# dominikh/jello

Hardware: AMD Instinct MI355X
Metric: Mpixels/sec fine-raster + paths/sec, 100k-path 4096^2 scene (higher is better)
Workload: dtype f32

## Files before the change

jello_amd/csrc/kernels_flatten.hip:

```cpp
#include <hip/hip_runtime.h>
__shared__ double fl_atan_tab[9];
#define JD_ATAN_TAB_LDS fl_atan_tab
#include "kcommon.h"
#define FF_INLINE __device__ __forceinline__
#include "flatten_fast.h"

using namespace jk;
using namespace jd;

namespace {

struct CubicParams { float th0, th1, chord_len, err; };
struct EulerParams { float th0, th1, k0, k1, ch; };
struct CubicPoints { V2 p0, p1, p2, p3; };
struct PointDeriv { V2 point, deriv; };
struct PathTagData { uint32_t tag_byte; MonoidK<5> monoid; };

#define DERIV_THRESH 1e-6f
#define DERIV_THRESH_SQUARED (DERIV_THRESH * DERIV_THRESH)
#define DERIV_EPS 1e-6f
#define SUBDIV_LIMIT (1.0f / 65536.0f)
#define K1_THRESH 1e-3f
#define DIST_THRESH 1e-3f
#define TANGENT_THRESH 1e-6f
// ... 684 lines not shown
            if (tag_monoids.ok(word_ix)) {
                store_tm(&tag_monoids.p[word_ix], pm);
            } else {
#pragma unroll
                for (int i = 0; i < 5; i++) pm.v[i] = 0u;
            }
            __syncthreads();
        } else {
            pm = load_tm(tag_monoids, word_ix);
        }
        const uint32_t ix0 = word_ix * 4u;
        for (uint32_t q = 0u; q < 12u; q++) {
            const uint32_t sl = ix0 * 3u + q;
            if (sl < cap) counts[sl] = 0u;
        }
        uint32_t th = 0u, tl = 0u;
#pragma unroll
        for (uint32_t k = 0; k < 4u; k++) {
            const uint32_t ix = ix0 + k;
            if (ix >= n_tags) continue;
            const MonoidK<5> tm = monoid_add(pm, reduce_tag(tag_word & ((1u << (k * 8u)) - 1u)));
            const uint32_t tag_byte = (tag_word >> (k * 8u)) & 0xffu;
            const uint32_t style_flags = scene.rd(cfg->layout.style_base + tm.v[3] - 2u);
            const bool is_stroke = (style_flags & JL_STYLE_FLAGS_STYLE) != 0u;
            const uint32_t path_ix = tm.v[4];
            if ((tag_byte & JL_PATH_TAG_PATH) != 0u && path_bboxes.ok(path_ix)) {
                path_bboxes.p[path_ix].draw_flags = ((style_flags & JL_STYLE_FLAGS_FILL) == 0u) ? 0u : 1u;
                path_bboxes.p[path_ix].trans_ix = tm.v[0] - 1u;
            }
            const uint32_t seg_type = tag_byte & JL_PATH_TAG_SEG_TYPE;
            const bool curved = seg_type != JL_PATH_TAG_LINETO;
            if (seg_type != 0u) {
                if (!is_stroke) {
                    if (curved) nh[blk][k] = 1u; else nl[blk][k] = 1u;
                } else if ((tag_byte & JL_PATH_TAG_SUBPATH_END) != 0u) {
                    if (curved) nl[blk][k] = 1u;
                } else {
                    if (curved) { nh[blk][k] = 2u; nl[blk][k] = 1u; } else { nl[blk][k] = 3u; }
                }
            }
            th += nh[blk][k];
            tl += nl[blk][k];
        }
        MonoidK<2> m, tot;
        m.v[0] = th; m.v[1] = tl;
        const MonoidK<2> e2 = block_excl_scan_monoid<2>(m, sh, &tot);
        eh[blk] = wg_h + e2.v[0];
        el[blk] = wg_l + e2.v[1];
        wg_h += tot.v[0];
        wg_l += tot.v[1];
        __syncthreads();
    }
    if (threadIdx.x == 0) {
        sh_base[0] = wg_h ? atomicAdd(&counters[0], wg_h) : 0u;
        sh_base[1] = wg_l ? atomicAdd(&counters[FL_CTR_LIGHT], wg_l) : 0u;
    }
    __syncthreads();
#pragma unroll
    for (uint32_t blk = 0; blk < PSC_BLOCKS; blk++) {
        const uint32_t ix0 = ((blockIdx.x * PSC_BLOCKS + blk) * JL_WG + threadIdx.x) * 4u;
        uint32_t ph = sh_base[0] + eh[blk], pl = sh_base[1] + el[blk];
#pragma unroll
        for (uint32_t k = 0; k < 4u; k++) {
            const uint32_t ix = ix0 + k;
            uint32_t sub = 0u;
            for (uint32_t q = 0; q < nh[blk][k]; q++, sub++, ph++)
                if (ph < cap) list[ph] = ix * 3u + sub;
            for (uint32_t q = 0; q < nl[blk][k]; q++, sub++, pl++)
                if (pl < cap) list[cap - 1u - pl] = ix * 3u + sub;
        }
    }
}

template <bool EMIT>
JD void run_item(const JlConfig* cfg, const Scene& s, Out<EMIT>& o, uint32_t slot, EulerJob& job, uint32_t& path_ix_out) {
    uint32_t ix = slot / 3u, sub = slot - ix * 3u;
    Seg g = load_seg(s, ix);
    uint32_t path_ix = g.tag.monoid.v[4];
    path_ix_out = path_ix;
    uint32_t style_ix = g.tag.monoid.v[3];
    uint32_t trans_ix = g.tag.monoid.v[0];
    uint32_t style_flags = g.style_flags;
    job.path_ix = path_ix; job.trans_ix = trans_ix;
    Xf transform;
    {
        uint32_t base = cfg->layout.transform_base + trans_ix * 6u;
        transform.m0 = u2f(s.scene.rd(base)); transform.m1 = u2f(s.scene.rd(base + 1u)); transform.m2 = u2f(s.scene.rd(base + 2u));
        transform.m3 = u2f(s.scene.rd(base + 3u)); transform.t0 = u2f(s.scene.rd(base + 4u)); transform.t1 = u2f(s.scene.rd(base + 5u));
    }
    CubicPoints pts = read_path_segment(s, g.tag, g.is_stroke);
    if (g.is_stroke) {
        float linewidth = u2f(s.scene.rd(cfg->layout.style_base + style_ix + 1u));
        float offset = 0.5f * linewidth;
        bool is_stroke_cap_marker = (g.tag.tag_byte & JL_PATH_TAG_SUBPATH_END) != 0u;
        if (is_stroke_cap_marker) {
            V2 tangent = cubic_start_tangent(pts.p0, pts.p1, pts.p2, pts.p3);
            V2 offset_tangent = offset * normalize(tangent);
            V2 n = v2(offset_tangent.y * -1.0f, offset_tangent.x * 1.0f);
            draw_cap<EMIT>(o, path_ix, (style_flags & JL_STYLE_FLAGS_START_CAP_MASK) >> 2, pts.p0, pts.p0 - n, pts.p0 + n, -offset_tangent,
                           transform);
        } else {
            const float TT = TANGENT_THRESH * TANGENT_THRESH;
            V2 tan_prev = cubic_end_tangent(pts.p0, pts.p1, pts.p2, pts.p3);
            if (dot(tan_prev, tan_prev) < TT) tan_prev = v2(TANGENT_THRESH, 0.0f);
            V2 offset_tangent = offset * normalize(tan_prev);
            V2 n_prev = v2(offset_tangent.y * -1.0f, offset_tangent.x * 1.0f);
            if (sub < 2u) {
                V2 tan_start = cubic_start_tangent(pts.p0, pts.p1, pts.p2, pts.p3);
                if (dot(tan_start, tan_start) < TT) tan_start = v2(TANGENT_THRESH, 0.0f);
                V2 n_start = offset * normalize(v2(-tan_start.y, tan_start.x));
                job.valid = true; job.cubic = pts; job.local_to_device = transform;
                if (sub == 0u) { job.offset = offset; job.start_p = pts.p0 + n_start; job.end_p = pts.p3 + n_prev; }
                else { job.offset = -offset; job.start_p = pts.p0 - n_start; job.end_p = pts.p3 - n_prev; }
            } else {
                PathTagData ntag = compute_tag_monoid(s, ix + 1u);
                CubicPoints npts = read_path_segment(s, ntag, true);
                bool n_is_closed = (ntag.tag_byte & JL_PATH_TAG_SEG_TYPE) == JL_PATH_TAG_LINETO;
                bool n_is_marker = (ntag.tag_byte & JL_PATH_TAG_SUBPATH_END) != 0u;
                bool do_join = !n_is_marker || n_is_closed;
                if (do_join) {
                    V2 tan_next = cubic_start_tangent(npts.p0, npts.p1, npts.p2, npts.p3);
                    if (dot(tan_next, tan_next) < TT) tan_next = v2(TANGENT_THRESH, 0.0f);
                    V2 tnn = normalize(tan_next);
                    V2 n_next = v2((offset * tnn.y) * -1.0f, (offset * tnn.x) * 1.0f);
                    draw_join<EMIT>(o, path_ix, style_flags, pts.p3, tan_prev, tan_next, n_prev, n_next, transform);
                } else {
                    draw_cap<EMIT>(o, path_ix, (style_flags & JL_STYLE_FLAGS_END_CAP_MASK), pts.p3, pts.p3 + n_prev, pts.p3 - n_prev, offset_tangent,
                                   transform);
                }
            }
        }
    } else {
        job.valid = true; job.cubic = pts; job.local_to_device = transform;
        job.offset = 0.0f; job.start_p = pts.p0; job.end_p = pts.p3;
    }
}

#ifndef FLQ_STACK
#define FLQ_STACK 448u
#endif
#ifndef FLQ_LEAVES
#define FLQ_LEAVES 640u
#endif
#ifndef FLQ_MAX_LEVEL
#define FLQ_MAX_LEVEL 9u
#endif
struct FlBatch {
    uint32_t jhead[64];
    uint32_t stack[FLQ_STACK];
    uint32_t l_tpos[FLQ_LEAVES];
    uint16_t l_key[FLQ_LEAVES];
    uint16_t l_link[FLQ_LEAVES];
    uint32_t unsure[128];
    uint32_t n_stack, n_leaves, bail, n_unsure;
};
JD float lanef(float v, uint32_t src) { return u2f((uint32_t)__builtin_amdgcn_ds_bpermute((int)(src << 2), (int)f2u(v))); }
JD uint32_t laneu(uint32_t v, uint32_t src) { return (uint32_t)__builtin_amdgcn_ds_bpermute((int)(src << 2), (int)v); }

struct NodeResult {
    bool accept;
    CubicParams cp;
    V2 es_p0, es_p1;
    bool ends_at_one;
};
struct NodeEnds {
    V2 last_p, last_q;
    float last_t;
    V2 point, deriv;
    float t1;
};
JD NodeEnds node_ends(V2 p0, V2 p1, V2 p2, V2 p3, uint32_t level, uint32_t t0_u) {
    const float dt = u2f((127u - level) << 23);
    const float t0 = (float)t0_u * dt;
    NodeEnds r;
    if (t0_u == 0u) {
        r.last_p = p0;
        r.last_q = p1 - p0;
        if (dot(r.last_q, r.last_q) < DERIV_THRESH_SQUARED) r.last_q = eval_cubic_and_deriv(p0, p1, p2, p3, DERIV_EPS).deriv;
        r.last_t = 0.0f;
    } else {
        PointDeriv pq0 = eval_cubic_and_deriv(p0, p1, p2, p3, t0);
        r.last_t = t0;
        if (dot(pq0.deriv, pq0.deriv) < DERIV_THRESH_SQUARED) {
            PointDeriv n0 = eval_cubic_and_deriv(p0, p1, p2, p3, t0 - DERIV_EPS);
            pq0.deriv = n0.deriv;
            pq0.point = n0.point;
            r.last_t = t0 - DERIV_EPS;
        }
        r.last_p = pq0.point;
        r.last_q = pq0.deriv;
    }
    float t1 = t0 + dt;
    PointDeriv this_pq1 = eval_cubic_and_deriv(p0, p1, p2, p3, t1);
    if (dot(this_pq1.deriv, this_pq1.deriv) < DERIV_THRESH_SQUARED) {
        PointDeriv new_pq1 = eval_cubic_and_deriv(p0, p1, p2, p3, t1 - DERIV_EPS);
        this_pq1.deriv = new_pq1.deriv;
        if (t1 < 1.0f) {
            this_pq1.point = new_pq1.point;
            t1 = t1 - DERIV_EPS;
        }
    }
    r.point = this_pq1.point;
    r.deriv = this_pq1.deriv;
    r.t1 = t1;
    return r;
}
JD NodeResult node_test(V2 p0, V2 p1, V2 p2, V2 p3, float scale, uint32_t level, uint32_t t0_u) {
    const float tol = 0.25f;
    const float dt = u2f((127u - level) << 23);
    const NodeEnds ne = node_ends(p0, p1, p2, p3, level, t0_u);
    const float actual_dt = ne.t1 - ne.last_t;
    NodeResult r;
    r.cp = cubic_from_points_derivs(ne.last_p, ne.point, ne.last_q, ne.deriv, actual_dt);
    r.accept = r.cp.err * scale <= tol || dt <= SUBDIV_LIMIT;
    r.es_p0 = ne.last_p;
    r.es_p1 = ne.point;
    r.ends_at_one = ne.t1 == 1.0f;
    return r;
}
JD int node_test_fast(V2 p0, V2 p1, V2 p2, V2 p3, float scale, uint32_t level, uint32_t t0_u, float* v_est, float* delta) {
    const float tol = 0.25f;
    const NodeEnds ne = node_ends(p0, p1, p2, p3, level, t0_u);
    const float actual_dt = ne.t1 - ne.last_t;
    const V2 chord = ne.point - ne.last_p;
    const float chord_squared = dot(chord, chord);
    const V2 q0 = ne.last_q, q1 = ne.deriv;
    *v_est = 0.0f; *delta = 0.0f;
    if (chord_squared < DERIV_THRESH_SQUARED) {
        const float chord_err = sqrt_((float)(9.0 / 32.0) * (dot(q0, q0) + dot(q1, q1))) * actual_dt;
        return (chord_err * scale <= tol) ? ffast::FF_ACCEPT : ffast::FF_REJECT;
    }
    const float chord_len = FF_SQRT(chord_squared);
    const float sc = actual_dt * FF_RCP(chord_squared);
    const V2 h0 = v2(q0.x * chord.x + q0.y * chord.y, q0.y * chord.x - q0.x * chord.y);
    const V2 h1 = v2(q1.x * chord.x + q1.y * chord.y, q1.x * chord.y - q1.y * chord.x);
    const float len0 = FF_SQRT(h0.x * h0.x + h0.y * h0.y), len1 = FF_SQRT(h1.x * h1.x + h1.y * h1.y);
    return ffast::ff_decide(h0.x, h0.y, len0, h1.x, h1.y, len1, len0 * sc, len1 * sc, chord_len, scale, tol, v_est, delta);
}
JD CubicParams piece_angles(const NodeEnds& ne) {
    const V2 chord = ne.point - ne.last_p;
    const float chord_squared = dot(chord, chord);
    CubicParams r;
    r.err = 0.0f;
    if (chord_squared < DERIV_THRESH_SQUARED) {
        r.th0 = 0.0f; r.th1 = 0.0f; r.chord_len = DERIV_THRESH;
        return r;
    }
    const V2 q0 = ne.last_q, q1 = ne.deriv;
    const V2 h0 = v2(q0.x * chord.x + q0.y * chord.y, q0.y * chord.x - q0.x * chord.y);
    const V2 h1 = v2(q1.x * chord.x + q1.y * chord.y, q1.x * chord.y - q1.y * chord.x);
    r.th0 = atan2_(h0.y, h0.x);
    r.th1 = atan2_(h1.y, h1.x);
    r.chord_len = sqrt_(chord_squared);
    return r;
}

struct PieceParams {
    EulerParams ep;
    float n, noff, int0, integral;
    uint32_t n_u, robust;
};
JD PieceParams piece_params(const CubicParams& cp, float scale, float offset) {
    const float tol = 0.25f;
    PieceParams r;
    r.ep = es_params_from_angles(cp.th0, cp.th1);
    const EulerParams& ep = r.ep;
    float k0 = ep.k0 - 0.5f * ep.k1;
    float k1 = ep.k1;
    float normalized_offset = offset / cp.chord_len;
    float dist_scaled = normalized_offset * ep.ch;
    float scale_multiplier = sqrt_(0.125f * scale * cp.chord_len / (ep.ch * tol));
    float a = 0.0f, b = 0.0f, integral = 0.0f, int0 = 0.0f, n_frac;
    uint32_t robust = 0u;
    if (abs_(k1) < K1_THRESH) {
        float k = ep.k0;
        n_frac = sqrt_(abs_(k * (k * dist_scaled + 1.0f)));
        robust = 1u;
    } else if (abs_(dist_scaled) < DIST_THRESH) {
        a = k1;
        b = k0;
        int0 = pow_1_5_signed(b);
        float int1 = pow_1_5_signed(a + b);
        integral = int1 - int0;
        n_frac = (float)(2.0 / 3.0) * integral / a;
        robust = 2u;
    } else {
        a = -2.0f * dist_scaled * k1;
        b = -1.0f - 2.0f * dist_scaled * k0;
        int0 = espc_int_approx(b);
        float int1 = espc_int_approx(a + b);
        integral = int1 - int0;
        float k_peak = k0 - k1 * b / a;
        float integrand_peak = sqrt_(abs_(k_peak * (k_peak * dist_scaled + 1.0f)));
        n_frac = integral * integrand_peak / a;
    }
    r.n = clamp_(ceil_(n_frac * scale_multiplier), 1.0f, 100.0f);
    r.n_u = to_u32(r.n);
    r.noff = normalized_offset;
    r.int0 = int0;
    r.integral = integral;
    r.robust = robust;
    return r;
}

#ifdef FL_FAST_CHECK
__device__ uint32_t g_ff_stats[8];
#endif
#ifndef FL_WAVES_PER_EU
#define FL_WAVES_PER_EU 4
#endif
#ifndef FL_BLOCKS_PER_CU
#define FL_BLOCKS_PER_CU 4
#endif
#ifdef FL_TIMING
#define FL_TL_WAVES 8192u
#define FL_TL_BATCHES 15u
#define FL_TL_WORDS (2u + 3u * FL_TL_BATCHES)
__device__ unsigned long long g_fl_timeline[FL_TL_WAVES * FL_TL_WORDS];
#endif
__global__ __launch_bounds__(JL_WG) __attribute__((amdgpu_waves_per_eu(FL_WAVES_PER_EU, FL_WAVES_PER_EU))) void k_flatten_items(const JlConfig* __restrict__ cfg, Buf<uint32_t> scene, Buf<JlTagMonoid> tag_monoids,
                                                         Buf<JlPathBbox> path_bboxes, const uint32_t* __restrict__ list,
                                                         uint32_t* __restrict__ counters, uint32_t cap, uint32_t* __restrict__ counts,
                                                         FlTemp T, uint32_t debug) {
    __shared__ FlBatch sh_batch[JL_WG / 64];
    Scene s;
    s.cfg = cfg; s.scene = scene; s.tag_monoids = tag_monoids;
    uint32_t n_heavy = umin_(counters[0], cap), n_light = umin_(counters[FL_CTR_LIGHT], cap - n_heavy);
    uint32_t n = n_heavy + n_light;
    const uint32_t units_h = n_heavy / 64u + (n_heavy % 64u != 0u ? 1u : 0u);
    const uint32_t units = units_h + n_light / 64u + (n_light % 64u != 0u ? 1u : 0u);
    const uint32_t n_groups = umin_(umax_(gridDim.x / FL_BLOCKS_PER_CU, 1u), FL_DEAL_GROUPS), group = blockIdx.x % n_groups;
    if (group >= units) return;
#ifdef FL_TIMING
    const unsigned long long tl_entry = wall_clock64();
    const uint32_t tl_wave = blockIdx.x * (JL_WG / 64u) + (threadIdx.x >> 6);
    uint32_t tl_n = 0u;
#endif
    atan_tab_fill();
    __syncthreads();
    const uint32_t lane = lane_id();
    FlBatch& B = sh_batch[threadIdx.x >> 6];
    Out<true> o;
    o.cfg = cfg; o.T = T; o.home_s = o.home_r = blockIdx.x % T.K; o.failed_s = o.failed_r = false; o.slot = 0u;
    if ((debug & 1u) != 0u) o.home_s = o.home_r = 0u;
#ifdef FL_SOAK_HOME0
    o.home_s = o.home_r = 0u;
#endif
    o.cursor = 0u; o.a_first = 0u; o.a_spos = 0u; o.a_rpos = 0u;
    for (;;) {
        uint32_t k = 0u;
        if (lane == 0u) k = atomicAdd(&counters[FL_CTR_DEAL + FL_DEAL_STRIDE * group], 1u);
        k = (uint32_t)__builtin_amdgcn_readfirstlane((int)k);
        const uint32_t u = k * n_groups + group;
        if (u >= units) break;
        const bool heavy = u < units_h;
        const uint32_t t_first = heavy ? u * 64u : n_heavy + (u - units_h) * 64u;
        const uint32_t t_end = umin_(t_first + 64u, heavy ? n_heavy : n);
        const uint32_t t = t_first + lane;
#ifdef FL_TIMING
        const unsigned long long tl_start = wall_clock64() | (heavy ? 1ull << 63 : 0ull);
        uint32_t tl_info = 0u;
#define FL_TL_END()                                                                                      \
    do {                                                                                                 \
        if (lane == 0u && tl_wave < FL_TL_WAVES && tl_n < FL_TL_BATCHES) {                               \
            g_fl_timeline[tl_wave * FL_TL_WORDS + 2u + 3u * tl_n] = tl_start;                            \
            g_fl_timeline[tl_wave * FL_TL_WORDS + 3u + 3u * tl_n] = wall_clock64();                      \
            g_fl_timeline[tl_wave * FL_TL_WORDS + 4u + 3u * tl_n] = tl_info;                             \
        }                                                                                                \
        tl_n++;                                                                                          \
    } while (0)
#else
#define FL_TL_END() do {} while (0)
#endif
        if (__builtin_amdgcn_ballot_w64(o.failed_s) != 0ull) { o.home_s = fl_next_home(T, o.home_s, 0); o.failed_s = false; }
        if (__builtin_amdgcn_ballot_w64(o.failed_r) != 0ull) { o.home_r = fl_next_home(T, o.home_r, 1); o.failed_r = false; }
        EulerJob job;
        job.valid = false; job.path_ix = 0u; job.trans_ix = 0u; job.offset = 0.0f;
        job.start_p = v2(0, 0); job.end_p = v2(0, 0);
        job.cubic.p0 = job.cubic.p1 = job.cubic.p2 = job.cubic.p3 = v2(0, 0);
        job.local_to_device = xf_identity();
        uint32_t slot = FL_INVALID;
        if (t < t_end) {
            slot = heavy ? list[t] : list[cap - 1u - (t - n_heavy)];
            o.slot = slot; o.cursor = 0u; o.a_first = 0u; o.a_spos = 0u; o.a_rpos = 0u;
            uint32_t path_ix;
            run_item<true>(cfg, s, o, slot, job, path_ix);
            if (!job.valid) counts[slot] = o.cursor;
        }
        EulerLane e;
        euler_begin(e, job);
        const bool active = job.valid && !e.done;
        if (__builtin_amdgcn_ballot_w64(active) == 0ull) {
            FL_TL_END();
            continue;
        }
        B.jhead[lane] = 0u;
        {
            const uint64_t am = __builtin_amdgcn_ballot_w64(active);
            if (active) B.stack[(uint32_t)__builtin_popcountll(am & ((1ull << lane) - 1ull))] = lane;
            if (lane == 0u) { B.n_stack = (uint32_t)__builtin_popcountll(am); B.n_leaves = 0u; B.bail = 0u; B.n_unsure = 0u; }
        }
        wave_fence();
#ifdef FL_SPLIT_NO_A
        if (lane == 0u) B.n_stack = 0u;
        wave_fence();
#endif
        for (;;) {
#ifdef FL_TIMING
            tl_info += 1u << 16;
#endif
            const uint32_t ns = (uint32_t)__builtin_amdgcn_readfirstlane((int)B.n_stack);
            const uint32_t nu = (uint32_t)__builtin_amdgcn_readfirstlane((int)B.n_unsure);
            if (ns == 0u && nu == 0u) break;
            const bool exact_round = ns == 0u || nu >= 64u;
            const uint32_t take = umin_(exact_round ? nu : ns, 64u);
            const bool has = lane < take;
            const uint32_t node = has ? (exact_round ? B.unsure[nu - 1u - lane] : B.stack[ns - 1u - lane]) : 0u;
            wave_fence();
            const uint32_t j = node & 63u, level = (node >> 6) & 31u, t0_u = node >> 11;
            const V2 jp0 = v2(lanef(e.p0.x, j), lanef(e.p0.y, j)), jp1 = v2(lanef(e.p1.x, j), lanef(e.p1.y, j));
            const V2 jp2 = v2(lanef(e.p2.x, j), lanef(e.p2.y, j)), jp3 = v2(lanef(e.p3.x, j), lanef(e.p3.y, j));
            const float scale = lanef(e.scale, j);
            int kind = ffast::FF_UNSURE;
            if (exact_round) {
                if (has) kind = node_test(jp0, jp1, jp2, jp3, scale, level, t0_u).accept ? ffast::FF_ACCEPT : ffast::FF_REJECT;
            } else if (has) {
                float v_est, delta;
                kind = node_test_fast(jp0, jp1, jp2, jp3, scale, level, t0_u, &v_est, &delta);
#ifdef FL_FAST_CHECK
            }
            if (!exact_round) {
                bool c_unsure = false, c_contra = false, c_viol = false;
                if (has) {
                    float v2_, d2_;
                    const int k2 = node_test_fast(jp0, jp1, jp2, jp3, scale, level, t0_u, &v2_, &d2_);
                    const NodeResult rx = node_test(jp0, jp1, jp2, jp3, scale, level, t0_u);
                    const float vx = rx.cp.err * scale;
                    c_unsure = k2 == ffast::FF_UNSURE;
                    c_contra = (k2 == ffast::FF_ACCEPT && !rx.accept) || (k2 == ffast::FF_REJECT && rx.accept);
                    c_viol = (d2_ > 0.0f && !(abs_(v2_ - vx) <= d2_)) || (d2_ == 0.0f && k2 != ffast::FF_UNSURE && v2_ != 0.0f);
                }
                const uint32_t n0 = (uint32_t)__builtin_popcountll(__builtin_amdgcn_ballot_w64(has));
                const uint32_t n1 = (uint32_t)__builtin_popcountll(__builtin_amdgcn_ballot_w64(c_unsure));
                const uint32_t n2 = (uint32_t)__builtin_popcountll(__builtin_amdgcn_ballot_w64(c_contra));
                const uint32_t n3 = (uint32_t)__builtin_popcountll(__builtin_amdgcn_ballot_w64(c_viol));
                if (lane == 0u) {
                    atomicAdd(&g_ff_stats[0], n0);
                    if (n1) atomicAdd(&g_ff_stats[1], n1);
                    if (n2) atomicAdd(&g_ff_stats[2], n2);
                    if (n3) atomicAdd(&g_ff_stats[3], n3);
                }
#endif
            }
            const bool acc = has && kind == ffast::FF_ACCEPT, rej = has && kind == ffast::FF_REJECT, uns = has && kind == ffast::FF_UNSURE;
            const uint64_t accm = __builtin_amdgcn_ballot_w64(acc), rejm = __builtin_amdgcn_ballot_w64(rej), unsm = __builtin_amdgcn_ballot_w64(uns);
            const uint32_t n_acc = (uint32_t)__builtin_popcountll(accm), n_rej = (uint32_t)__builtin_popcountll(rejm);
            const uint32_t n_uns = (uint32_t)__builtin_popcountll(unsm);
            const uint32_t nl = (uint32_t)__builtin_amdgcn_readfirstlane((int)B.n_leaves);
            const uint32_t ns_left = exact_round ? ns : ns - take, nu_left = exact_round ? nu - take : nu;
            const bool too_deep = __builtin_amdgcn_ballot_w64(rej && level + 1u > FLQ_MAX_LEVEL) != 0ull;
            if (too_deep || ns_left + 2u * n_rej > FLQ_STACK || nl + n_acc > FLQ_LEAVES) {
                if (lane == 0u) B.bail = 1u;
                wave_fence();
                break;
            }
            const uint64_t below = (1ull << lane) - 1ull;
            if (rej) {
                const uint32_t pos = ns_left + 2u * (uint32_t)__builtin_popcountll(rejm & below);
                B.stack[pos] = j | ((level + 1u) << 6) | ((2u * t0_u + 1u) << 11);
                B.stack[pos + 1u] = j | ((level + 1u) << 6) | ((2u * t0_u) << 11);
            }
            if (acc) {
                const uint32_t li = nl + (uint32_t)__builtin_popcountll(accm & below);
                B.l_tpos[li] = node;
                B.l_key[li] = (uint16_t)((t0_u << (FLQ_MAX_LEVEL - level)) << 7);
                const uint32_t prev = atomicExch(&B.jhead[j], li + 1u);
                B.l_link[li] = (uint16_t)((j << 10) | prev);
            }
            if (uns) B.unsure[nu_left + (uint32_t)__builtin_popcountll(unsm & below)] = node;
            if (lane == 0u) { B.n_stack = ns_left + 2u * n_rej; B.n_leaves = nl + n_acc; B.n_unsure = nu_left + n_uns; }
            wave_fence();
        }
        const bool bail = (uint32_t)__builtin_amdgcn_readfirstlane((int)B.bail) != 0u;
        const uint32_t nl = bail ? 0u : (uint32_t)__builtin_amdgcn_readfirstlane((int)B.n_leaves);
#ifdef FL_TIMING
        tl_info = (tl_info & 0x7fff0000u) | (nl & 0xffffu) | (bail ? 1u << 31 : 0u);
#endif
        uint32_t rec_base = 0u;
        if (nl != 0u && lane == 0u) rec_base = fl_grab<1>(T, o.home_r, nl, o.failed_r);
        rec_base = (uint32_t)__builtin_amdgcn_readlane((int)rec_base, 0);
#ifdef FL_SPLIT_NO_B
        for (uint32_t lbase = nl; lbase < nl; lbase += 64u) {
#else
        for (uint32_t lbase = 0u; lbase < nl; lbase += 64u) {
#endif
            const uint32_t li = lbase + lane;
            const bool has = li < nl;
            const uint32_t node = has ? B.l_tpos[li] : 0u;
            const uint32_t j = node & 63u, level = (node >> 6) & 31u, t0_u = node >> 11;
            const V2 jp0 = v2(lanef(e.p0.x, j), lanef(e.p0.y, j)), jp1 = v2(lanef(e.p1.x, j), lanef(e.p1.y, j));
            const V2 jp2 = v2(lanef(e.p2.x, j), lanef(e.p2.y, j)), jp3 = v2(lanef(e.p3.x, j), lanef(e.p3.y, j));
            const float scale = lanef(e.scale, j), offset = lanef(e.offset, j);
            const uint32_t j_slot = laneu(slot, j), j_path = laneu(e.path_ix, j), j_trans = laneu(e.trans_ix, j);
            const float j_tsx = lanef(e.t_start.x, j), j_tsy = lanef(e.t_start.y, j), j_tex = lanef(e.t_end.x, j), j_tey = lanef(e.t_end.y, j);
            if (has) {
                const NodeEnds ne = node_ends(jp0, jp1, jp2, jp3, level, t0_u);
                const CubicParams cp = piece_angles(ne);
                const PieceParams pp = piece_params(cp, scale, offset);
                const uint32_t fl = pp.robust | ((ne.t1 == 1.0f) ? 4u : 0u) | ((offset >= 0.0f) ? 8u : 0u) | ((offset == 0.0f) ? 16u : 0u) |
                                    ((t0_u == 0u) ? 32u : 0u);
                const uint32_t r = rec_base + li;
                if (rec_base != FL_INVALID)
                    piece_record_write(T.recs + (size_t)r * 4u, ne.last_p, ne.point, pp.ep.th0, pp.ep.th1, pp.int0, pp.integral, pp.noff, j_slot, j_path,
                                       j_trans, fl, 0u, v2(j_tsx, j_tsy), v2(j_tex, j_tey));
                B.l_key[li] = (uint16_t)(B.l_key[li] | pp.n_u);
            }
        }
        wave_fence();
        if (nl != 0u) {
            uint32_t total = 0u;
            if (active)
                for (uint32_t q = B.jhead[lane]; q != 0u; q = B.l_link[q - 1u] & 1023u) total += B.l_key[q - 1u] & 127u;
            if (active) counts[slot] = total;
            const uint32_t incl = wave_incl_scan_u32(total);
            const uint32_t batch_total = (uint32_t)__builtin_amdgcn_readlane((int)incl, 63);
            const bool together = batch_total <= ((debug & 4u) != 0u ? 48u : FL_MAX_GRAB);
            uint32_t grab = 0u;
            if (together) {
                if (lane == 0u) grab = fl_grab<0>(T, o.home_s, batch_total, o.failed_s);
            } else if (active && total != 0u) {
                grab = fl_grab<0>(T, o.home_s, total, o.failed_s);
            }
            for (uint32_t li = lane; li < nl; li += 64u) {
                const uint32_t j = B.l_link[li] >> 10, key = B.l_key[li];
                uint32_t first = 0u;
                for (uint32_t q = B.jhead[j]; q != 0u; q = B.l_link[q - 1u] & 1023u) {
                    const uint32_t k2 = B.l_key[q - 1u];
                    if ((k2 >> 7) < (key >> 7)) first += k2 & 127u;
                }
                B.l_tpos[li] = first;
            }
            {
                const uint32_t base0 = (uint32_t)__builtin_amdgcn_readlane((int)grab, 0);
                B.unsure[lane] = together ? (base0 == FL_INVALID ? FL_INVALID : base0 + (incl - total)) : grab;
            }
            wave_fence();
            for (uint32_t li = lane; li < nl; li += 64u) {
                const uint32_t j = B.l_link[li] >> 10, key = B.l_key[li], first = B.l_tpos[li];
                const uint32_t r = rec_base + li, jb = B.unsure[j];
                if (rec_base != FL_INVALID && (key >> 7) != 0u) ((uint32_t*)T.recs)[(size_t)r * 16u + 12u] = first;
                if (jb == FL_INVALID) continue;
                if (rec_base != FL_INVALID) piece_slots_write(T.sinfo, jb + first, key & 127u, r);
                else for (uint32_t i = 0u; i < (key & 127u); i++) T.sinfo[jb + first + i] = make_uint2(0u, 0u);
            }
            wave_fence();
        }
        if (__builtin_expect(bail, 0)) {
            o.slot = slot; o.cursor = 0u; o.a_first = 0u; o.a_spos = 0u; o.a_rpos = 0u;
            bool have = active;
            auto finish = [&]() -> bool {
                if (e.done && have) {
                    counts[o.slot] = o.cursor;
                    have = false;
                }
                return __builtin_amdgcn_ballot_w64(!e.done) != 0ull;
            };
            flatten_euler_wave(o, e, finish);
        }
        FL_TL_END();
    }
#ifdef FL_TIMING
    if (lane == 0u && tl_wave < FL_TL_WAVES) {
        g_fl_timeline[tl_wave * FL_TL_WORDS] = tl_entry;
        g_fl_timeline[tl_wave * FL_TL_WORDS + 1u] = tl_n;
    }
#endif
#undef FL_TL_END
}

#ifndef FL_LINES_WAVES_PER_EU
#define FL_LINES_WAVES_PER_EU 4
#endif
__global__ __launch_bounds__(JL_WG) __attribute__((amdgpu_waves_per_eu(FL_LINES_WAVES_PER_EU, FL_LINES_WAVES_PER_EU))) void k_flatten_lines(const JlConfig* __restrict__ cfg, Buf<uint32_t> scene, const uint32_t* __restrict__ counters,
                                                         FlTemp T, const uint32_t* __restrict__ bases, uint32_t n_slots, Buf<JlLineSoup> lines) {
    atan_tab_fill();
    const uint32_t lines_lim = umin_(cfg->lines_size, lines.n);
    const uint2* __restrict__ sinfo = T.sinfo;
    const uint4* __restrict__ recs = T.recs;
    const uint32_t n_r = T.K * T.R;
    uint32_t ru[FL_MAX_REGIONS], used[FL_MAX_REGIONS];
    uint32_t units = 0u;
#pragma unroll
    for (uint32_t c = 0u; c < FL_MAX_REGIONS; c++) {
        ru[c] = units;
        used[c] = c < T.K ? umin_(counters[FL_CTR_CURSOR + FL_CUR_STRIDE * c], T.R) : 0u;
        units += (used[c] + JL_WG - 1u) / JL_WG;
    }
    auto fetch_info = [&](uint32_t u) -> uint2 {
        if (u >= units) return make_uint2(0u, 0u);
        uint32_t c = 0u, first_unit = 0u, in_use = used[0];
#pragma unroll
        for (uint32_t q = 1u; q < FL_MAX_REGIONS; q++)
            if (u >= ru[q] && used[q] != 0u) { c = q; first_unit = ru[q]; in_use = used[q]; }
        const uint32_t in_region = (u - first_unit) * JL_WG + threadIdx.x;
        return in_region < in_use ? sinfo[(size_t)c * T.R + in_region] : make_uint2(0u, 0u);
    };
    auto state_of = [&](uint2 si) -> uint32_t {
        if (si.x >= n_r) return 0u;
        return (si.y & FL_INFO_PIECE) != 0u ? 2u : ((si.y & FL_INFO_DIRECT) != 0u ? 1u : 0u);
    };
    auto fetch_rec = [&](uint32_t state, uint32_t r, uint4& r0, uint4& r1, uint4& r2, uint4& r3) {
        r0 = r1 = r2 = r3 = make_uint4(0u, 0u, 0u, 0u);
        const uint4* rec = recs + (size_t)r * 4u;
        if (state != 0u) { r0 = rec[0]; r1 = rec[1]; }
        if (state == 2u) { r2 = rec[2]; r3 = rec[3]; }
    };
    const uint32_t G = gridDim.x;
    uint2 si_a = fetch_info(blockIdx.x), si_b = fetch_info(blockIdx.x + G);
    uint32_t st_a = state_of(si_a);
    uint4 a0, a1, a2, a3;
    fetch_rec(st_a, si_a.x, a0, a1, a2, a3);
    for (uint32_t u = blockIdx.x; u < units; u += G) {
        const uint32_t st = st_a;
        const uint2 si = si_a;
        const uint4 r0 = a0, r1 = a1, r2 = a2, r3 = a3;
        si_a = si_b;
        st_a = state_of(si_a);
        fetch_rec(st_a, si_a.x, a0, a1, a2, a3);
        si_b = fetch_info(u + 2u * G);
        uint32_t widx[3] = {0xffffffffu, 0xffffffffu, 0xffffffffu};
        uint2 wdat[3] = {make_uint2(0u, 0u), make_uint2(0u, 0u), make_uint2(0u, 0u)};
        if (st == 1u) {
            const uint32_t item = r0.x, k = r0.y;
            if (item < n_slots) {
                const uint32_t dst = bases[item] + k;
                if (dst < lines_lim) {
                    widx[0] = dst * 3u; wdat[0] = make_uint2(r0.z, 0u);
                    widx[1] = dst * 3u + 1u; wdat[1] = make_uint2(r1.x, r1.y);
                    widx[2] = dst * 3u + 2u; wdat[2] = make_uint2(r1.z, r1.w);
                }
            }
        } else if (st == 2u) {
            const uint32_t n_u = (si.y >> 8) & 127u, i = si.y & 127u;
            const uint32_t flags = r2.w & 63u;
            const bool last_of_item = i + 1u == n_u && (flags & 4u) != 0u;
            const uint32_t slot = r2.y, k = ((flags & 32u) != 0u ? 0u : r3.x) + i;
            Xf tr;
            if ((flags & 16u) != 0u) {
                tr = xf_identity();
            } else {
                uint32_t tb = cfg->layout.transform_base + (r2.w >> 6) * 6u;
                tr.m0 = u2f(scene.rd(tb)); tr.m1 = u2f(scene.rd(tb + 1u)); tr.m2 = u2f(scene.rd(tb + 2u));
                tr.m3 = u2f(scene.rd(tb + 3u)); tr.t0 = u2f(scene.rd(tb + 4u)); tr.t1 = u2f(scene.rd(tb + 5u));
            }
            const uint32_t slot_base = slot < n_slots ? bases[slot] : 0u;
            V2 lp1;
            if (last_of_item) {
                lp1 = v2(u2f(r3.z), u2f(r3.w));
#if defined(FL_LSPLIT) && FL_LSPLIT == 1
            } else if (true) {
                lp1 = v2(u2f(r0.x) + (float)i, u2f(r0.w) + u2f(r1.x) + u2f(r1.y) + u2f(r1.z) + u2f(r1.w) + u2f(r2.x));
#endif
            } else {
                const EulerParams ep = es_params_from_angles(u2f(r1.x), u2f(r1.y));
                const float noff = u2f(r2.x), n = (float)n_u;
                const float tt = (float)(i + 1u) / n;
                float sarg = tt;
                const uint32_t robust = flags & 3u;
                if (robust != 1u) {
                    const float k0 = ep.k0 - 0.5f * ep.k1, k1 = ep.k1;
                    const float dist_scaled = noff * ep.ch;
                    const float int0 = u2f(r1.z), integral = u2f(r1.w);
                    float a, b;
                    if (robust == 2u) {
                        a = k1;
                        b = k0;
                    } else {
                        a = -2.0f * dist_scaled * k1;
                        b = -1.0f - 2.0f * dist_scaled * k0;
                    }
                    float uu = integral * tt + int0;
                    float inv;
                    if (robust == 2u) inv = pow23_abs_(uu) * sign_(uu); else inv = espc_int_inv_approx(uu);
                    sarg = (inv - b) / a;
                }
                lp1 = es_seg_eval_with_offset(v2(u2f(r0.x), u2f(r0.y)), v2(u2f(r0.z), u2f(r0.w)), ep, sarg, noff);
            }
            const V2 q = xf_apply(tr, lp1);
            if (slot < n_slots) {
                const uint32_t dst = slot_base + k;
                const bool fwd = (flags & 8u) != 0u;
                const bool has_next = !last_of_item && dst + 1u < lines_lim;
                const uint2 hdr = make_uint2(r2.z, 0u), pt = make_uint2(f2u(q.x), f2u(q.y));
                if (dst < lines_lim) {
                    if (k == 0u) {
                        uint2* w = (uint2*)lines.p;
                        const V2 qs = xf_apply(tr, v2(u2f(r3.x), u2f(r3.y)));
                        w[(size_t)dst * 3u] = hdr;
                        w[(size_t)dst * 3u + (fwd ? 1u : 2u)] = make_uint2(f2u(qs.x), f2u(qs.y));
                    }
                    widx[0] = dst * 3u + (fwd ? 2u : 1u); wdat[0] = pt;
                    if (has_next) {
// ... 263 lines not shown
```

Before: 20930.

## Share subdivision tree between paired stroke sides in batched flatten

Detects adjacent lanes whose slots form a stroke pair (same cubic with opposite offsets) and lets only the first lane drive the adaptive subdivision tree, tagging its nodes with a pair bit. Accepted leaves of paired trees are emitted twice into a split leaf array (pairs from the front, singles from the back), and the per-leaf endpoint/angle/Euler parameters are computed once and reused for both offsets. This removes duplicated subdivision and curve-fitting work for stroke sides, at the cost of more complex leaf indexing, an extra inner loop over sides, and an assumption that paired sides always subdivide identically.

```diff
diff --git a/jello_amd/csrc/kernels_flatten.hip b/jello_amd/csrc/kernels_flatten.hip
--- a/jello_amd/csrc/kernels_flatten.hip
+++ b/jello_amd/csrc/kernels_flatten.hip
@@ -860,7 +860,7 @@
     uint16_t l_key[FLQ_LEAVES];
     uint16_t l_link[FLQ_LEAVES];
     uint32_t unsure[128];
-    uint32_t n_stack, n_leaves, bail, n_unsure;
+    uint32_t n_stack, n_pairs, n_single, bail, n_unsure;
 };
 JD float lanef(float v, uint32_t src) { return u2f((uint32_t)__builtin_amdgcn_ds_bpermute((int)(src << 2), (int)f2u(v))); }
 JD uint32_t laneu(uint32_t v, uint32_t src) { return (uint32_t)__builtin_amdgcn_ds_bpermute((int)(src << 2), (int)v); }
@@ -968,16 +968,27 @@
     float n, noff, int0, integral;
     uint32_t n_u, robust;
 };
-JD PieceParams piece_params(const CubicParams& cp, float scale, float offset) {
+struct PieceShared {
+    EulerParams ep;
+    float chord_len, scale_multiplier;
+};
+JD PieceShared piece_shared(const CubicParams& cp, float scale) {
     const float tol = 0.25f;
+    PieceShared r;
+    r.ep = es_params_from_angles(cp.th0, cp.th1);
+    r.chord_len = cp.chord_len;
+    r.scale_multiplier = sqrt_(0.125f * scale * cp.chord_len / (r.ep.ch * tol));
+    return r;
+}
+JD PieceParams piece_params(const PieceShared& ps, float offset) {
     PieceParams r;
-    r.ep = es_params_from_angles(cp.th0, cp.th1);
+    r.ep = ps.ep;
     const EulerParams& ep = r.ep;
     float k0 = ep.k0 - 0.5f * ep.k1;
     float k1 = ep.k1;
-    float normalized_offset = offset / cp.chord_len;
+    float normalized_offset = offset / ps.chord_len;
     float dist_scaled = normalized_offset * ep.ch;
-    float scale_multiplier = sqrt_(0.125f * scale * cp.chord_len / (ep.ch * tol));
+    float scale_multiplier = ps.scale_multiplier;
     float a = 0.0f, b = 0.0f, integral = 0.0f, int0 = 0.0f, n_frac;
     uint32_t robust = 0u;
     if (abs_(k1) < K1_THRESH) {
@@ -1067,7 +1078,7 @@
         const uint32_t t = t_first + lane;
 #ifdef FL_TIMING
         const unsigned long long tl_start = wall_clock64() | (heavy ? 1ull << 63 : 0ull);
-        uint32_t tl_info = 0u;
+        unsigned long long tl_info = 0u;
 #define FL_TL_END()                                                                                      \
     do {                                                                                                 \
         if (lane == 0u && tl_wave < FL_TL_WAVES && tl_n < FL_TL_BATCHES) {                               \
@@ -1105,8 +1116,13 @@
         B.jhead[lane] = 0u;
         {
             const uint64_t am = __builtin_amdgcn_ballot_w64(active);
-            if (active) B.stack[(uint32_t)__builtin_popcountll(am & ((1ull << lane) - 1ull))] = lane;
-            if (lane == 0u) { B.n_stack = (uint32_t)__builtin_popcountll(am); B.n_leaves = 0u; B.bail = 0u; B.n_unsure = 0u; }
+            const uint32_t slot_before = laneu(slot, (lane + 63u) & 63u);
+            const bool second = active && lane != 0u && slot - (slot / 3u) * 3u == 1u && slot_before + 1u == slot && ((am >> (lane - 1u)) & 1ull) != 0ull;
+            const uint64_t secm = __builtin_amdgcn_ballot_w64(second), rootm = am & ~secm;
+            const bool two = (((secm >> 1) >> lane) & 1ull) != 0ull;
+            if (active && !second)
+                B.stack[(uint32_t)__builtin_popcountll(rootm & ((1ull << lane) - 1ull))] = lane | (two ? 0x80000000u : 0u);
+            if (lane == 0u) { B.n_stack = (uint32_t)__builtin_popcountll(rootm); B.n_pairs = 0u; B.n_single = 0u; B.bail = 0u; B.n_unsure = 0u; }
         }
         wave_fence();
 #ifdef FL_SPLIT_NO_A
@@ -1123,9 +1139,12 @@
             const bool exact_round = ns == 0u || nu >= 64u;
             const uint32_t take = umin_(exact_round ? nu : ns, 64u);
             const bool has = lane < take;
+#ifdef FL_TIMING
+            if (!exact_round) tl_info += (unsigned long long)take << 32;
+#endif
             const uint32_t node = has ? (exact_round ? B.unsure[nu - 1u - lane] : B.stack[ns - 1u - lane]) : 0u;
             wave_fence();
-            const uint32_t j = node & 63u, level = (node >> 6) & 31u, t0_u = node >> 11;
+            const uint32_t j = node & 63u, level = (node >> 6) & 31u, t0_u = (node >> 11) & 0xfffffu;
             const V2 jp0 = v2(lanef(e.p0.x, j), lanef(e.p0.y, j)), jp1 = v2(lanef(e.p1.x, j), lanef(e.p1.y, j));
             const V2 jp2 = v2(lanef(e.p2.x, j), lanef(e.p2.y, j)), jp3 = v2(lanef(e.p3.x, j), lanef(e.p3.y, j));
             const float scale = lanef(e.scale, j);
@@ -1164,10 +1183,13 @@
             const uint64_t accm = __builtin_amdgcn_ballot_w64(acc), rejm = __builtin_amdgcn_ballot_w64(rej), unsm = __builtin_amdgcn_ballot_w64(uns);
             const uint32_t n_acc = (uint32_t)__builtin_popcountll(accm), n_rej = (uint32_t)__builtin_popcountll(rejm);
             const uint32_t n_uns = (uint32_t)__builtin_popcountll(unsm);
-            const uint32_t nl = (uint32_t)__builtin_amdgcn_readfirstlane((int)B.n_leaves);
+            const bool acc2 = acc && (node >> 31) != 0u;
+            const uint64_t acc2m = __builtin_amdgcn_ballot_w64(acc2), acc1m = accm & ~acc2m;
+            const uint32_t n_acc2 = (uint32_t)__builtin_popcountll(acc2m);
+            const uint32_t n2 = (uint32_t)__builtin_amdgcn_readfirstlane((int)B.n_pairs), n1 = (uint32_t)__builtin_amdgcn_readfirstlane((int)B.n_single);
             const uint32_t ns_left = exact_round ? ns : ns - take, nu_left = exact_round ? nu - take : nu;
             const bool too_deep = __builtin_amdgcn_ballot_w64(rej && level + 1u > FLQ_MAX_LEVEL) != 0ull;
-            if (too_deep || ns_left + 2u * n_rej > FLQ_STACK || nl + n_acc > FLQ_LEAVES) {
+            if (too_deep || ns_left + 2u * n_rej > FLQ_STACK || 2u * n2 + n1 + n_acc + n_acc2 > FLQ_LEAVES) {
                 if (lane == 0u) B.bail = 1u;
                 wave_fence();
                 break;
@@ -1175,53 +1197,76 @@
             const uint64_t below = (1ull << lane) - 1ull;
             if (rej) {
                 const uint32_t pos = ns_left + 2u * (uint32_t)__builtin_popcountll(rejm & below);
-                B.stack[pos] = j | ((level + 1u) << 6) | ((2u * t0_u + 1u) << 11);
-                B.stack[pos + 1u] = j | ((level + 1u) << 6) | ((2u * t0_u) << 11);
+                const uint32_t tree = (node & 0x80000000u) | j | ((level + 1u) << 6);
+                B.stack[pos] = tree | ((2u * t0_u + 1u) << 11);
+                B.stack[pos + 1u] = tree | ((2u * t0_u) << 11);
             }
             if (acc) {
-                const uint32_t li = nl + (uint32_t)__builtin_popcountll(accm & below);
+                const uint32_t li = acc2 ? 2u * (n2 + (uint32_t)__builtin_popcountll(acc2m & below))
+                                         : FLQ_LEAVES - 1u - (n1 + (uint32_t)__builtin_popcountll(acc1m & below));
+                const uint16_t key = (uint16_t)((t0_u << (FLQ_MAX_LEVEL - level)) << 7);
                 B.l_tpos[li] = node;
-                B.l_key[li] = (uint16_t)((t0_u << (FLQ_MAX_LEVEL - level)) << 7);
+                B.l_key[li] = key;
                 const uint32_t prev = atomicExch(&B.jhead[j], li + 1u);
                 B.l_link[li] = (uint16_t)((j << 10) | prev);
+                if (acc2) {
+                    B.l_key[li + 1u] = key;
+                    const uint32_t prev1 = atomicExch(&B.jhead[j + 1u], li + 2u);
+                    B.l_link[li + 1u] = (uint16_t)(((j + 1u) << 10) | prev1);
+                }
             }
             if (uns) B.unsure[nu_left + (uint32_t)__builtin_popcountll(unsm & below)] = node;
-            if (lane == 0u) { B.n_stack = ns_left + 2u * n_rej; B.n_leaves = nl + n_acc; B.n_unsure = nu_left + n_uns; }
+            if (lane == 0u) { B.n_stack = ns_left + 2u * n_rej; B.n_pairs = n2 + n_acc2; B.n_single = n1 + n_acc - n_acc2; B.n_unsure = nu_left + n_uns; }
             wave_fence();
         }
         const bool bail = (uint32_t)__builtin_amdgcn_readfirstlane((int)B.bail) != 0u;
-        const uint32_t nl = bail ? 0u : (uint32_t)__builtin_amdgcn_readfirstlane((int)B.n_leaves);
+        const uint32_t n2 = bail ? 0u : (uint32_t)__builtin_amdgcn_readfirstlane((int)B.n_pairs);
+        const uint32_t n1 = bail ? 0u : (uint32_t)__builtin_amdgcn_readfirstlane((int)B.n_single);
+        const uint32_t nl = 2u * n2 + n1;
 #ifdef FL_TIMING
-        tl_info = (tl_info & 0x7fff0000u) | (nl & 0xffffu) | (bail ? 1u << 31 : 0u);
+        tl_info = (tl_info & 0xffffffff7fff0000ull) | (nl & 0xffffu) | (bail ? 1ull << 31 : 0ull);
 #endif
         uint32_t rec_base = 0u;
         if (nl != 0u && lane == 0u) rec_base = fl_grab<1>(T, o.home_r, nl, o.failed_r);
         rec_base = (uint32_t)__builtin_amdgcn_readlane((int)rec_base, 0);
 #ifdef FL_SPLIT_NO_B
-        for (uint32_t lbase = nl; lbase < nl; lbase += 64u) {
+        for (uint32_t lbase = n2 + n1; lbase < n2 + n1; lbase += 64u) {
 #else
-        for (uint32_t lbase = 0u; lbase < nl; lbase += 64u) {
-#endif
-            const uint32_t li = lbase + lane;
-            const bool has = li < nl;
+        for (uint32_t lbase = 0u; lbase < n2 + n1; lbase += 64u) {
+#endif
+            const uint32_t v = lbase + lane;
+            const bool has = v < n2 + n1, pair = v < n2;
+            const uint32_t li = pair ? 2u * v : FLQ_LEAVES - 1u - (v - n2);
             const uint32_t node = has ? B.l_tpos[li] : 0u;
-            const uint32_t j = node & 63u, level = (node >> 6) & 31u, t0_u = node >> 11;
+            const uint32_t j = node & 63u, level = (node >> 6) & 31u, t0_u = (node >> 11) & 0xfffffu;
             const V2 jp0 = v2(lanef(e.p0.x, j), lanef(e.p0.y, j)), jp1 = v2(lanef(e.p1.x, j), lanef(e.p1.y, j));
             const V2 jp2 = v2(lanef(e.p2.x, j), lanef(e.p2.y, j)), jp3 = v2(lanef(e.p3.x, j), lanef(e.p3.y, j));
-            const float scale = lanef(e.scale, j), offset = lanef(e.offset, j);
-            const uint32_t j_slot = laneu(slot, j), j_path = laneu(e.path_ix, j), j_trans = laneu(e.trans_ix, j);
-            const float j_tsx = lanef(e.t_start.x, j), j_tsy = lanef(e.t_start.y, j), j_tex = lanef(e.t_end.x, j), j_tey = lanef(e.t_end.y, j);
+            const float scale = lanef(e.scale, j);
+            NodeEnds ne;
+            PieceShared ps;
+            ne.last_p = ne.last_q = ne.point = ne.deriv = v2(0, 0); ne.last_t = ne.t1 = 0.0f;
+            ps.ep.th0 = ps.ep.th1 = ps.ep.k0 = ps.ep.k1 = ps.ep.ch = 0.0f; ps.chord_len = ps.scale_multiplier = 0.0f;
             if (has) {
-                const NodeEnds ne = node_ends(jp0, jp1, jp2, jp3, level, t0_u);
-                const CubicParams cp = piece_angles(ne);
-                const PieceParams pp = piece_params(cp, scale, offset);
-                const uint32_t fl = pp.robust | ((ne.t1 == 1.0f) ? 4u : 0u) | ((offset >= 0.0f) ? 8u : 0u) | ((offset == 0.0f) ? 16u : 0u) |
-                                    ((t0_u == 0u) ? 32u : 0u);
-                const uint32_t r = rec_base + li;
-                if (rec_base != FL_INVALID)
-                    piece_record_write(T.recs + (size_t)r * 4u, ne.last_p, ne.point, pp.ep.th0, pp.ep.th1, pp.int0, pp.integral, pp.noff, j_slot, j_path,
-                                       j_trans, fl, 0u, v2(j_tsx, j_tsy), v2(j_tex, j_tey));
-                B.l_key[li] = (uint16_t)(B.l_key[li] | pp.n_u);
+                ne = node_ends(jp0, jp1, jp2, jp3, level, t0_u);
+                ps = piece_shared(piece_angles(ne), scale);
+            }
+            const uint32_t sides = lbase < n2 ? 2u : 1u;
+            for (uint32_t side = 0u; side < sides; side++) {
+                const bool hs = has && (side == 0u || pair);
+                const uint32_t js = (j + side) & 63u;
+                const float offset = lanef(e.offset, js);
+                const uint32_t j_slot = laneu(slot, js), j_path = laneu(e.path_ix, js), j_trans = laneu(e.trans_ix, js);
+                const float j_tsx = lanef(e.t_start.x, js), j_tsy = lanef(e.t_start.y, js), j_tex = lanef(e.t_end.x, js), j_tey = lanef(e.t_end.y, js);
+                if (hs) {
+                    const PieceParams pp = piece_params(ps, offset);
+                    const uint32_t fl = pp.robust | ((ne.t1 == 1.0f) ? 4u : 0u) | ((offset >= 0.0f) ? 8u : 0u) | ((offset == 0.0f) ? 16u : 0u) |
+                                        ((t0_u == 0u) ? 32u : 0u);
+                    const uint32_t r = rec_base + (pair ? li + side : 2u * n2 + (v - n2));
+                    if (rec_base != FL_INVALID)
+                        piece_record_write(T.recs + (size_t)r * 4u, ne.last_p, ne.point, pp.ep.th0, pp.ep.th1, pp.int0, pp.integral, pp.noff, j_slot, j_path,
+                                           j_trans, fl, 0u, v2(j_tsx, j_tsy), v2(j_tex, j_tey));
+                    B.l_key[li + side] = (uint16_t)(B.l_key[li + side] | pp.n_u);
+                }
             }
         }
         wave_fence();
@@ -1239,7 +1284,8 @@
             } else if (active && total != 0u) {
                 grab = fl_grab<0>(T, o.home_s, total, o.failed_s);
             }
-            for (uint32_t li = lane; li < nl; li += 64u) {
+            for (uint32_t y = lane; y < nl; y += 64u) {
+                const uint32_t li = y < 2u * n2 ? y : FLQ_LEAVES - 1u - (y - 2u * n2);
                 const uint32_t j = B.l_link[li] >> 10, key = B.l_key[li];
                 uint32_t first = 0u;
                 for (uint32_t q = B.jhead[j]; q != 0u; q = B.l_link[q - 1u] & 1023u) {
@@ -1253,9 +1299,10 @@
                 B.unsure[lane] = together ? (base0 == FL_INVALID ? FL_INVALID : base0 + (incl - total)) : grab;
             }
             wave_fence();
-            for (uint32_t li = lane; li < nl; li += 64u) {
+            for (uint32_t y = lane; y < nl; y += 64u) {
+                const uint32_t li = y < 2u * n2 ? y : FLQ_LEAVES - 1u - (y - 2u * n2);
                 const uint32_t j = B.l_link[li] >> 10, key = B.l_key[li], first = B.l_tpos[li];
-                const uint32_t r = rec_base + li, jb = B.unsure[j];
+                const uint32_t r = rec_base + y, jb = B.unsure[j];
                 if (rec_base != FL_INVALID && (key >> 7) != 0u) ((uint32_t*)T.recs)[(size_t)r * 16u + 12u] = first;
                 if (jb == FL_INVALID) continue;
                 if (rec_base != FL_INVALID) piece_slots_write(T.sinfo, jb + first, key & 127u, r);
```

Result: no change. 20920 (-0.1%).
